# adrianstanea/UnitSpeech

Measured on AMD Instinct MI355X. Metric: mel-frames/sec @ 50 diffusion steps, 80x1024, higher is better.
Workload: dtype f32; 1 GPU; B=1 utterance(s)/GPU, 80x1024 mel, 50 diffusion steps, text+spk CFG (3 score evals/step), full-size decoder (119.1M params, synthetic weights), built-in Philox noise; batch_per_gpu=1, frames=1024, diffusion_steps=50, parallelism=utterance-sharded x1

## Files before the change

unitspeech_amd/csrc/wino4.hip:

```cpp
#include "kernels.h"
#include "pack_f16.h"
#include "wino4_coef.h"

namespace us {

typedef float f32x4 __attribute__((ext_vector_type(4)));
typedef _Float16 half4w __attribute__((ext_vector_type(4)));

namespace {

template <int M> struct Coef;
template <> struct Coef<4> {
  static constexpr int N = 6;
  static constexpr float bt(int i, int j) { return wino4::kBT4[i][j]; }
  static constexpr float at(int i, int j) { return wino4::kAT4[i][j]; }
  static constexpr double g(int i, int j) { return wino4::kG4[i][j]; }
};
template <> struct Coef<2> {
  static constexpr int N = 4;
  static constexpr float bt(int i, int j) { return wino4::kBT2[i][j]; }
  static constexpr float at(int i, int j) { return wino4::kAT2[i][j]; }
  static constexpr double g(int i, int j) { return wino4::kG2[i][j]; }
};

__device__ __forceinline__ void axpy(f32x4& acc, float c, const f32x4& x, bool& first) {
  if (c == 0.f) return;
  if (first) { acc = c == 1.f ? x : (c == -1.f ? -x : x * c); first = false; return; }
  if (c == 1.f) acc += x;
  else if (c == -1.f) acc -= x;
  else acc += x * c;
}

constexpr float kVScale = 0x1p-5f, kVUnscale = 0x1p+5f;

template <int M> struct Bt;
template <> struct Bt<4> {
  __device__ static __forceinline__ void apply(const f32x4 (&d)[6], f32x4 (&o)[6]) {
    using K = Coef<4>;
    static_assert(K::bt(2, 1) == -K::bt(1, 1) && K::bt(2, 3) == -K::bt(1, 3) && K::bt(2, 2) == K::bt(1, 2) && K::bt(1, 4) == 1.f, "symmetric points");
    static_assert(K::bt(4, 1) == -K::bt(3, 1) && K::bt(4, 3) == -K::bt(3, 3) && K::bt(4, 2) == K::bt(3, 2) && K::bt(3, 4) == 1.f, "symmetric points");
    static_assert(K::bt(0, 4) == 1.f && K::bt(5, 5) == 1.f && K::bt(0, 1) == 0.f && K::bt(0, 3) == 0.f && K::bt(5, 2) == 0.f && K::bt(5, 4) == 0.f, "layout");
    o[0] = d[0] * K::bt(0, 0) + (d[2] * K::bt(0, 2) + d[4]);
    o[5] = d[1] * K::bt(5, 1) + (d[3] * K::bt(5, 3) + d[5]);
    const f32x4 e1 = d[2] * K::bt(1, 2) + d[4], o1 = d[1] * K::bt(1, 1) + d[3] * K::bt(1, 3);
    o[1] = e1 + o1;
    o[2] = e1 - o1;
    const f32x4 e2 = d[2] * K::bt(3, 2) + d[4], o2 = d[1] * K::bt(3, 1) + d[3] * K::bt(3, 3);
    o[3] = e2 + o2;
    o[4] = e2 - o2;
  }
};
template <> struct Bt<2> {
  __device__ static __forceinline__ void apply(const f32x4 (&d)[4], f32x4 (&o)[4]) {
    using K = Coef<2>;
    static_assert(K::bt(0, 0) == -1.f && K::bt(0, 2) == 1.f && K::bt(1, 1) == 1.f && K::bt(1, 2) == 1.f && K::bt(2, 1) == -1.f && K::bt(2, 2) == 1.f &&
                      K::bt(3, 1) == -1.f && K::bt(3, 3) == 1.f, "F(2, 3) on {0, +-1, inf}");
    o[0] = d[2] - d[0];
    o[1] = d[2] + d[1];
    o[2] = d[2] - d[1];
    o[3] = d[3] - d[1];
  }
};

template <int MH, int MW, bool GN>
__global__ __launch_bounds__(256) void wino4_input_kernel(const float* __restrict__ x, int x_ld, float* __restrict__ V, int B, int H, int W,
                                                          int C, WinoGnArgs g, unsigned* range_flag) {
  constexpr int NH = Coef<MH>::N, NW = Coef<MW>::N;
  const int C4 = C >> 2;
  const int th = (H + MH - 1) / MH, tw = (W + MW - 1) / MW;
  const int b = blockIdx.y;
  const unsigned per_item = (unsigned)th * tw * C4;
  const long long plane_h = 2LL * B * th * tw * C;
  const unsigned item_bytes = (unsigned)H * W * x_ld * 4u;
  __amdgpu_buffer_rsrc_t rx = __builtin_amdgcn_make_buffer_rsrc((void*)(x + (long long)b * H * W * x_ld), 0, (int)item_bytes, 0x00020000);
  const float* mb = GN ? g.mask + (long long)(b % g.mask_bmod) * g.mask_ld : nullptr;
  const int cg = C / kGroups;
  _Float16* vb = reinterpret_cast<_Float16*>(V) + 2LL * (long long)b * th * tw * C;
  int tc = -1;
  f32x4 sc = {0.f, 0.f, 0.f, 0.f}, sh = sc, te = sc;
  float amax = 0.f;
  for (unsigned i = blockIdx.x * 256u + threadIdx.x; i < per_item; i += gridDim.x * 256u) {
    const unsigned t = i / C4;
    const int c = (int)(i - t * C4) * 4;
    const int ty = (int)(t / tw), tx = (int)(t - (unsigned)ty * tw);
    if (GN && tc != c) {
      tc = c;
      const double cnt = (double)H * W * cg;
      const double mean = stat_read(g.stats, b, c / cg, 0) / cnt;
      double var = stat_read(g.stats, b, c / cg, 1) / cnt - mean * mean;
      if (var < 0) var = 0;
      const float meanf = (float)mean, rstd = (float)(1.0 / sqrt(var + 1e-5));
      const f32x4 ga = *reinterpret_cast<const f32x4*>(g.gamma + c), be = *reinterpret_cast<const f32x4*>(g.beta + c);
      sc = ga * rstd;
      sh = be - sc * meanf;
      te = g.temb ? *reinterpret_cast<const f32x4*>(g.temb + (long long)b * C + c) : f32x4{0.f, 0.f, 0.f, 0.f};
      te *= kVScale;
    }
    unsigned coff[NW];
    float cm[NW];
#pragma unroll
    for (int q = 0; q < NW; ++q) {
      const int ix = MW * tx - 1 + q;
      const bool ok = (unsigned)ix < (unsigned)W;
      coff[q] = ok ? ((unsigned)ix * (unsigned)x_ld + (unsigned)c) * 4u : 0x80000000u;
      if (GN) cm[q] = ok ? mb[ix * g.mask_step] : 0.f;
    }
    f32x4 tr[NH][NW];
#pragma unroll
    for (int r = 0; r < NH; ++r) {
      const int iy = MH * ty - 1 + r;
      const bool rok = (unsigned)iy < (unsigned)H;
      const unsigned roff = rok ? (unsigned)iy * (unsigned)W * (unsigned)x_ld * 4u : 0x80000000u;
      f32x4 d[NW];
#pragma unroll
      for (int q = 0; q < NW; ++q) {
        f32x4 v = __builtin_bit_cast(f32x4, __builtin_amdgcn_raw_buffer_load_b128(rx, (int)((roff + (coff[q] & 0x7fffffffu)) | (coff[q] & 0x80000000u)), 0, 0));
        if (GN) {
          const float m = rok ? cm[q] : 0.f;
#pragma unroll
          for (int k = 0; k < 4; ++k) {
            const float z = v[k] * sc[k] + sh[k];
            const float w = __expf(z);
            const float u = w * (w + 2.f);
            const float mi = z > 20.f ? z : z * (u * __builtin_amdgcn_rcpf(u + 2.f));
            v[k] = (mi * (m * kVScale) + te[k]) * m;
          }
        } else {
          v *= kVScale;
        }
        d[q] = v;
      }
      Bt<MW>::apply(d, tr[r]);
    }
    const unsigned vo = ((unsigned)(ty * tw + tx) * (unsigned)C + (unsigned)c);
    const unsigned ho = 2u * (vo & ~7u) + (vo & 7u);
#pragma unroll
    for (int j = 0; j < NW; ++j) {
      f32x4 col[NH], vv[NH];
#pragma unroll
      for (int r = 0; r < NH; ++r) col[r] = tr[r][j];
      Bt<MH>::apply(col, vv);
#pragma unroll
      for (int ii = 0; ii < NH; ++ii) {
        half4w hi, lo;
#pragma unroll
        for (int k = 0; k < 4; ++k) {
          const float xv = vv[ii][k];
          amax = fmaxf(amax, fabsf(xv));
          const us_half h = (us_half)xv;
          hi[k] = h;
          lo[k] = (us_half)((xv - (float)h) * 2048.f);
        }
        _Float16* pf = vb + (long long)(ii * NW + j) * plane_h;
        *reinterpret_cast<half4w*>(pf + ho) = hi;
        *reinterpret_cast<half4w*>(pf + ho + 8) = lo;
      }
    }
  }
  range_report(range_flag, amax >= kF16Over, kRangeAct);
}

template <int MH, int MW>
__global__ __launch_bounds__(256) void wino4_output_kernel(const float* __restrict__ M, const float* __restrict__ bias, float* __restrict__ out,
                                                           int out_ld, double* __restrict__ stats, int B, int H, int W, int C) {
  using CH = Coef<MH>;
  using CW = Coef<MW>;
  constexpr int NH = CH::N, NW = CW::N;
  __shared__ double s_g[kGroups][2];
  const int C4 = C >> 2;
  const int th = (H + MH - 1) / MH, tw = (W + MW - 1) / MW;
  const int b = blockIdx.y;
  const long long per_item = (long long)th * tw * C4;
  const long long plane = (long long)B * th * tw * C;
  const int cg = C / kGroups;
  if (threadIdx.x < kGroups * 2) s_g[threadIdx.x >> 1][threadIdx.x & 1] = 0.0;
  __syncthreads();
  double t1[4] = {0, 0, 0, 0}, t2[4] = {0, 0, 0, 0};
  int tc = -1;
  auto flush = [&]() {
    if (tc >= 0) {
#pragma unroll
      for (int k = 0; k < 4; ++k) {
        atomicAdd(&s_g[(tc + k) / cg][0], t1[k]);
        atomicAdd(&s_g[(tc + k) / cg][1], t2[k]);
        t1[k] = t2[k] = 0;
      }
    }
  };
  for (unsigned i = blockIdx.x * 256u + threadIdx.x; i < (unsigned)per_item; i += gridDim.x * 256u) {
    const unsigned t = i / (unsigned)C4;
    const int c = (int)(i - t * (unsigned)C4) * 4;
    const int ty = (int)(t / (unsigned)tw);
    const int tx = (int)(t - (unsigned)ty * (unsigned)tw);
    const float* mb = M + (((long long)b * th + ty) * tw + tx) * C + c;
    f32x4 y[MH][MW];
#pragma unroll
    for (int r = 0; r < MH; ++r)
#pragma unroll
      for (int q = 0; q < MW; ++q) y[r][q] = f32x4{0.f, 0.f, 0.f, 0.f};
#pragma unroll
    for (int fi = 0; fi < NH; ++fi) {
      f32x4 m[NW];
#pragma unroll
      for (int fj = 0; fj < NW; ++fj) m[fj] = *reinterpret_cast<const f32x4*>(mb + (long long)(fi * NW + fj) * plane);
#pragma unroll
      for (int q = 0; q < MW; ++q) {
        f32x4 u = {0.f, 0.f, 0.f, 0.f};
        bool first = true;
#pragma unroll
        for (int fj = 0; fj < NW; ++fj) axpy(u, CW::at(q, fj), m[fj], first);
#pragma unroll
        for (int r = 0; r < MH; ++r) {
          bool never = false;
          axpy(y[r][q], CH::at(r, fi), u, never);
        }
      }
    }
    f32x4 bv = {0.f, 0.f, 0.f, 0.f};
    if (bias) bv = *reinterpret_cast<const f32x4*>(bias + c);
    if (stats && tc != c) { flush(); tc = c; }
    float* ob = out + (long long)b * H * W * out_ld + c;
#pragma unroll
    for (int r = 0; r < MH; ++r)
#pragma unroll
      for (int q = 0; q < MW; ++q) {
        const int oy = MH * ty + r, ox = MW * tx + q;
        if (oy < H && ox < W) {
          const f32x4 v = y[r][q] * kVUnscale + bv;
          *reinterpret_cast<f32x4*>(ob + ((long long)oy * W + ox) * out_ld) = v;
          if (stats) {
#pragma unroll
            for (int k = 0; k < 4; ++k) { t1[k] += (double)v[k]; t2[k] += (double)(v[k] * v[k]); }
          }
        }
      }
  }
  if (stats) {
    const int seg = C4 / kGroups;
    const bool wave_merge = (((long long)gridDim.x * 256) % C4) == 0 && seg >= 1 && seg <= 64 && (seg & (seg - 1)) == 0 && (64 % seg) == 0 &&
                            (C4 % 64 == 0 || 64 % C4 == 0);
    if (wave_merge) {
      double s1 = (t1[0] + t1[1]) + (t1[2] + t1[3]), s2 = (t2[0] + t2[1]) + (t2[2] + t2[3]);
      for (int off = 1; off < seg; off <<= 1) {
        s1 += __shfl_xor(s1, off);
        s2 += __shfl_xor(s2, off);
      }
      const int lane = threadIdx.x & 63;
      if ((lane & (seg - 1)) == 0 && tc >= 0) {
        atomicAdd(&s_g[tc / cg][0], s1);
        atomicAdd(&s_g[tc / cg][1], s2);
      }
    } else {
      flush();
    }
    __syncthreads();
    if (threadIdx.x < kGroups * 2)
      stat_add(stats, b, threadIdx.x >> 1, threadIdx.x & 1, blockIdx.x, s_g[threadIdx.x >> 1][threadIdx.x & 1]);
  }
}

template <int MH, int MW>
__global__ __launch_bounds__(256) void wino4_pack_kernel(const float* __restrict__ src, _Float16* __restrict__ dst, int Cout, int Cin,
                                                         unsigned* range_flag) {
  using CH = Coef<MH>;
  using CW = Coef<MW>;
  constexpr int NH = CH::N, NW = CW::N;
  bool over = false;
  const long long total = (long long)(Cin / 8) * Cout;
  const long long fstride = (long long)Cin * Cout * 2;
  for (long long i = blockIdx.x * 256LL + threadIdx.x; i < total; i += (long long)gridDim.x * 256) {
    const int g4 = (int)(i & 3);
    const long long rn = i >> 2;
    const int n = (int)(rn % Cout), kc = (int)(rn / Cout);
    const int k0 = kc * 32 + g4 * 8;
    float gk[8][9];
#pragma unroll
    for (int kk = 0; kk < 8; ++kk) {
      const float* gs = src + ((long long)n * Cin + k0 + kk) * 9;
#pragma unroll
      for (int t = 0; t < 9; ++t) gk[kk][t] = gs[t];
    }
    _Float16* d = dst + (rn * 32 + g4 * 8) * 2;
#pragma unroll
    for (int fi = 0; fi < NH; ++fi)
#pragma unroll
      for (int fj = 0; fj < NW; ++fj) {
        pk_half8 hi, lo;
#pragma unroll
        for (int kk = 0; kk < 8; ++kk) {
          double u = 0.0;
#pragma unroll
          for (int a = 0; a < 3; ++a)
#pragma unroll
            for (int bb = 0; bb < 3; ++bb) {
              const double cf = CH::g(fi, a) * CW::g(fj, bb);
              if (cf != 0.0) u += cf * (double)gk[kk][a * 3 + bb];
            }
          us_half h, l;
          split_f16x3((float)u, h, l, over);
          hi[kk] = h;
          lo[kk] = l;
        }
        *reinterpret_cast<pk_half8*>(d + (long long)(fi * NW + fj) * fstride) = hi;
        *reinterpret_cast<pk_half8*>(d + (long long)(fi * NW + fj) * fstride + 8) = lo;
      }
  }
  range_report(range_flag, over, kRangeWeight);
}

int grid_for(long long per_item) {
  long long blocks = (per_item + 255) / 256;
  return (int)(blocks < 1 ? 1 : (blocks > 4096 ? 4096 : blocks));
}

}

bool wino4_form_ok(int form) { return form == 44 || form == 24; }
int wino4_freqs(int form) { return form == 44 ? 36 : (form == 24 ? 24 : 0); }
void wino4_tiles(int form, int H, int W, int* th, int* tw) {
  const int mh = form / 10, mw = form % 10;
  *th = (H + mh - 1) / mh;
  *tw = (W + mw - 1) / mw;
}

hipError_t launch_wino4_input(int form, const float* x, int x_ld, float* V, int B, int H, int W, int C, const WinoGnArgs* gn, hipStream_t s) {
  if (!wino4_form_ok(form) || C % 8 != 0 || x_ld % 4 != 0 || B > 65535) return hipErrorInvalidValue;
  if ((long long)H * W * x_ld * 4 >= (1LL << 31) || (long long)H * W * C >= (1LL << 30)) return hipErrorInvalidValue;
  WinoGnArgs g{};
  if (gn) {
    g = *gn;
    if (!g.stats || !g.gamma || !g.beta || !g.mask || g.h_out || x_ld != C || C % kGroups != 0 || (C / kGroups) % 4 != 0) return hipErrorInvalidValue;
    if (g.mask_bmod < 1) g.mask_bmod = 1;
  }
  int th, tw;
  wino4_tiles(form, H, W, &th, &tw);
  const dim3 grid(grid_for((long long)th * tw * (C / 4)), B);
  unsigned* rf = current_range_flag();
  if (form == 44) {
    if (gn) hipLaunchKernelGGL((wino4_input_kernel<4, 4, true>), grid, dim3(256), 0, s, x, x_ld, V, B, H, W, C, g, rf);
    else hipLaunchKernelGGL((wino4_input_kernel<4, 4, false>), grid, dim3(256), 0, s, x, x_ld, V, B, H, W, C, g, rf);
  } else {
    if (gn) hipLaunchKernelGGL((wino4_input_kernel<2, 4, true>), grid, dim3(256), 0, s, x, x_ld, V, B, H, W, C, g, rf);
    else hipLaunchKernelGGL((wino4_input_kernel<2, 4, false>), grid, dim3(256), 0, s, x, x_ld, V, B, H, W, C, g, rf);
  }
  return hipGetLastError();
}

hipError_t launch_wino4_output(int form, const float* M, const float* bias, float* out, int out_ld, double* stats, int B, int H, int W, int C,
                               hipStream_t s) {
  if (!wino4_form_ok(form) || C % 4 != 0 || out_ld % 4 != 0 || C % kGroups != 0 || B > 65535) return hipErrorInvalidValue;
  int th, tw;
  wino4_tiles(form, H, W, &th, &tw);
  if ((long long)th * tw * (C / 4) >= (1LL << 31)) return hipErrorInvalidValue;
  const dim3 grid(grid_for((long long)th * tw * (C / 4)), B);
  if (form == 44) hipLaunchKernelGGL((wino4_output_kernel<4, 4>), grid, dim3(256), 0, s, M, bias, out, out_ld, stats, B, H, W, C);
  else hipLaunchKernelGGL((wino4_output_kernel<2, 4>), grid, dim3(256), 0, s, M, bias, out, out_ld, stats, B, H, W, C);
  return hipGetLastError();
}

hipError_t launch_wino4_pack_weight(int form, const float* src, float* dst, int Cout, int Cin, hipStream_t s) {
  if (!wino4_form_ok(form) || Cin % 32 != 0) return hipErrorInvalidValue;
  const long long total = (long long)Cout * Cin / 8;
  long long blocks = (total + 255) / 256;
  if (blocks > 8192) blocks = 8192;
  unsigned* rf = current_range_flag();
  if (form == 44) hipLaunchKernelGGL((wino4_pack_kernel<4, 4>), dim3((int)blocks), dim3(256), 0, s, src, reinterpret_cast<_Float16*>(dst), Cout, Cin, rf);
  else hipLaunchKernelGGL((wino4_pack_kernel<2, 4>), dim3((int)blocks), dim3(256), 0, s, src, reinterpret_cast<_Float16*>(dst), Cout, Cin, rf);
  return hipGetLastError();
}

}
```

Baseline: 3205 mel-frames/s.

## Stage Winograd input patches in LDS and pair hi/lo stores via permlane swap

The Winograd input transform now gives each workgroup a spatial patch of tiles plus a 32-channel slab. It loads the overlapping halo region once into shared memory, applying GroupNorm+Mish there, instead of each thread reloading overlapping 6x6 windows from global memory and recomputing the activation per overlap. Lanes in the two wave halves swap hi/lo f16 halves with permlane32_swap so each lane writes one 16-byte store instead of two 8-byte stores. This adds LDS use, a barrier, a fixed grid shape and FP-contract control in the Bt transform, which may affect occupancy and numerics.

```diff
diff --git a/unitspeech_amd/csrc/wino4.hip b/unitspeech_amd/csrc/wino4.hip
--- a/unitspeech_amd/csrc/wino4.hip
+++ b/unitspeech_amd/csrc/wino4.hip
@@ -2,10 +2,14 @@
 #include "pack_f16.h"
 #include "wino4_coef.h"
 
+#include <type_traits>
+
 namespace us {
 
 typedef float f32x4 __attribute__((ext_vector_type(4)));
 typedef _Float16 half4w __attribute__((ext_vector_type(4)));
+typedef unsigned u32x2 __attribute__((ext_vector_type(2)));
+typedef unsigned u32x4 __attribute__((ext_vector_type(4)));
 
 namespace {
 
@@ -35,13 +39,24 @@
 
 template <int M> struct Bt;
 template <> struct Bt<4> {
+  template <bool kScaledInput = false>
   __device__ static __forceinline__ void apply(const f32x4 (&d)[6], f32x4 (&o)[6]) {
     using K = Coef<4>;
     static_assert(K::bt(2, 1) == -K::bt(1, 1) && K::bt(2, 3) == -K::bt(1, 3) && K::bt(2, 2) == K::bt(1, 2) && K::bt(1, 4) == 1.f, "symmetric points");
     static_assert(K::bt(4, 1) == -K::bt(3, 1) && K::bt(4, 3) == -K::bt(3, 3) && K::bt(4, 2) == K::bt(3, 2) && K::bt(3, 4) == 1.f, "symmetric points");
     static_assert(K::bt(0, 4) == 1.f && K::bt(5, 5) == 1.f && K::bt(0, 1) == 0.f && K::bt(0, 3) == 0.f && K::bt(5, 2) == 0.f && K::bt(5, 4) == 0.f, "layout");
     o[0] = d[0] * K::bt(0, 0) + (d[2] * K::bt(0, 2) + d[4]);
-    o[5] = d[1] * K::bt(5, 1) + (d[3] * K::bt(5, 3) + d[5]);
+    if constexpr (kScaledInput) {
+      f32x4 t;
+      {
+#pragma clang fp contract(off)
+        const f32x4 p = d[3] * K::bt(5, 3);
+        t = p + d[5];
+      }
+      o[5] = d[1] * K::bt(5, 1) + t;
+    } else {
+      o[5] = d[1] * K::bt(5, 1) + (d[3] * K::bt(5, 3) + d[5]);
+    }
     const f32x4 e1 = d[2] * K::bt(1, 2) + d[4], o1 = d[1] * K::bt(1, 1) + d[3] * K::bt(1, 3);
     o[1] = e1 + o1;
     o[2] = e1 - o1;
@@ -62,29 +77,59 @@
   }
 };
 
+template <int MH, int MW> struct Patch {
+  static constexpr int PH = MH == 4 ? 2 : 5, PW = 8;
+  static constexpr int RH = PH * MH + 2, RW = PW * MW + 2;
+  static constexpr int kPix = RH * RW;
+  static constexpr int kSlab = 32;
+  static constexpr int kPixStride = 9;
+  static constexpr int kThreads = PH * 64;
+  static constexpr int kIter = (kPix * 8 + kThreads - 1) / kThreads;
+  static_assert(kPix * kPixStride * 16 <= 64 * 1024, "two workgroups share a CU's LDS");
+};
+
 template <int MH, int MW, bool GN>
-__global__ __launch_bounds__(256) void wino4_input_kernel(const float* __restrict__ x, int x_ld, float* __restrict__ V, int B, int H, int W,
-                                                          int C, WinoGnArgs g, unsigned* range_flag) {
+__global__ __launch_bounds__((Patch<MH, MW>::kThreads)) void wino4_input_kernel(const float* __restrict__ x, int x_ld, float* __restrict__ V, int B,
+                                                                               int H, int W, int C, WinoGnArgs g, unsigned* range_flag, int slabs,
+                                                                               int patches_w) {
+  using P = Patch<MH, MW>;
   constexpr int NH = Coef<MH>::N, NW = Coef<MW>::N;
-  const int C4 = C >> 2;
+  __shared__ f32x4 s_d[P::kPix * P::kPixStride];
   const int th = (H + MH - 1) / MH, tw = (W + MW - 1) / MW;
   const int b = blockIdx.y;
-  const unsigned per_item = (unsigned)th * tw * C4;
+  const int slab = (int)(blockIdx.x % (unsigned)slabs);
+  const int patch = (int)(blockIdx.x / (unsigned)slabs);
+  const int pty = patch / patches_w, ptx = patch - pty * patches_w;
+  const int tid = threadIdx.x;
   const long long plane_h = 2LL * B * th * tw * C;
   const unsigned item_bytes = (unsigned)H * W * x_ld * 4u;
   __amdgpu_buffer_rsrc_t rx = __builtin_amdgcn_make_buffer_rsrc((void*)(x + (long long)b * H * W * x_ld), 0, (int)item_bytes, 0x00020000);
-  const float* mb = GN ? g.mask + (long long)(b % g.mask_bmod) * g.mask_ld : nullptr;
-  const int cg = C / kGroups;
   _Float16* vb = reinterpret_cast<_Float16*>(V) + 2LL * (long long)b * th * tw * C;
-  int tc = -1;
-  f32x4 sc = {0.f, 0.f, 0.f, 0.f}, sh = sc, te = sc;
-  float amax = 0.f;
-  for (unsigned i = blockIdx.x * 256u + threadIdx.x; i < per_item; i += gridDim.x * 256u) {
-    const unsigned t = i / C4;
-    const int c = (int)(i - t * C4) * 4;
-    const int ty = (int)(t / tw), tx = (int)(t - (unsigned)ty * tw);
-    if (GN && tc != c) {
-      tc = c;
+  {
+    const int q = tid & 7;
+    const int c = slab * P::kSlab + q * 4;
+    const bool cok = c < C;
+    const int slot = (q >> 1) + 4 * (q & 1);
+    const float* mb = GN ? g.mask + (long long)(b % g.mask_bmod) * g.mask_ld : nullptr;
+    const int y0 = pty * (P::PH * MH) - 1, x0 = ptx * (P::PW * MW) - 1;
+    f32x4 v[P::kIter];
+    float pm[P::kIter];
+#pragma unroll
+    for (int k = 0; k < P::kIter; ++k) {
+      const int p = (tid + k * P::kThreads) >> 3;
+      const int py = p / P::RW, px = p - py * P::RW;
+      const int iy = y0 + py, ix = x0 + px;
+      const bool ok = cok && (unsigned)iy < (unsigned)H && (unsigned)ix < (unsigned)W && p < P::kPix;
+      const unsigned off = ok ? (((unsigned)iy * (unsigned)W + (unsigned)ix) * (unsigned)x_ld + (unsigned)c) * 4u : 0x80000000u;
+      v[k] = __builtin_bit_cast(f32x4, __builtin_amdgcn_raw_buffer_load_b128(rx, (int)off, 0, 0));
+      if (GN) {
+        const float mv = mb[min(max(ix, 0), W - 1) * g.mask_step];
+        pm[k] = ok ? mv : 0.f;
+      }
+    }
+    f32x4 sc = {0.f, 0.f, 0.f, 0.f}, sh = sc, te = sc;
+    if (GN && cok) {
+      const int cg = C / kGroups;
       const double cnt = (double)H * W * cg;
       const double mean = stat_read(g.stats, b, c / cg, 0) / cnt;
       double var = stat_read(g.stats, b, c / cg, 1) / cnt - mean * mean;
@@ -96,44 +141,44 @@
       te = g.temb ? *reinterpret_cast<const f32x4*>(g.temb + (long long)b * C + c) : f32x4{0.f, 0.f, 0.f, 0.f};
       te *= kVScale;
     }
-    unsigned coff[NW];
-    float cm[NW];
-#pragma unroll
-    for (int q = 0; q < NW; ++q) {
-      const int ix = MW * tx - 1 + q;
-      const bool ok = (unsigned)ix < (unsigned)W;
-      coff[q] = ok ? ((unsigned)ix * (unsigned)x_ld + (unsigned)c) * 4u : 0x80000000u;
-      if (GN) cm[q] = ok ? mb[ix * g.mask_step] : 0.f;
-    }
+#pragma unroll
+    for (int k = 0; k < P::kIter; ++k) {
+      const int p = (tid + k * P::kThreads) >> 3;
+      f32x4 d = v[k];
+      if (GN) {
+        const float m = pm[k];
+#pragma unroll
+        for (int kk = 0; kk < 4; ++kk) {
+          const float z = d[kk] * sc[kk] + sh[kk];
+          const float w = __expf(z);
+          const float u = w * (w + 2.f);
+          const float mi = z > 20.f ? z : z * (u * __builtin_amdgcn_rcpf(u + 2.f));
+          d[kk] = (mi * (m * kVScale) + te[kk]) * m;
+        }
+      } else {
+        d *= kVScale;
+      }
+      if (p < P::kPix) s_d[p * P::kPixStride + slot] = d;
+    }
+  }
+  __syncthreads();
+  const int lane = tid & 63, trow = tid >> 6;
+  const int tcol = (lane & 31) >> 2, oct = lane & 3, odd = lane >> 5;
+  const int ty = pty * P::PH + trow, tx = ptx * P::PW + tcol;
+  const int c8 = slab * P::kSlab + oct * 8;
+  float amax = 0.f;
+  if (ty < th && tx < tw && c8 < C) {
+    const f32x4* sp = s_d + ((trow * MH) * P::RW + tcol * MW) * P::kPixStride + oct + 4 * odd;
     f32x4 tr[NH][NW];
 #pragma unroll
     for (int r = 0; r < NH; ++r) {
-      const int iy = MH * ty - 1 + r;
-      const bool rok = (unsigned)iy < (unsigned)H;
-      const unsigned roff = rok ? (unsigned)iy * (unsigned)W * (unsigned)x_ld * 4u : 0x80000000u;
       f32x4 d[NW];
 #pragma unroll
-      for (int q = 0; q < NW; ++q) {
-        f32x4 v = __builtin_bit_cast(f32x4, __builtin_amdgcn_raw_buffer_load_b128(rx, (int)((roff + (coff[q] & 0x7fffffffu)) | (coff[q] & 0x80000000u)), 0, 0));
-        if (GN) {
-          const float m = rok ? cm[q] : 0.f;
-#pragma unroll
-          for (int k = 0; k < 4; ++k) {
-            const float z = v[k] * sc[k] + sh[k];
-            const float w = __expf(z);
-            const float u = w * (w + 2.f);
-            const float mi = z > 20.f ? z : z * (u * __builtin_amdgcn_rcpf(u + 2.f));
-            v[k] = (mi * (m * kVScale) + te[k]) * m;
-          }
-        } else {
-          v *= kVScale;
-        }
-        d[q] = v;
-      }
-      Bt<MW>::apply(d, tr[r]);
-    }
-    const unsigned vo = ((unsigned)(ty * tw + tx) * (unsigned)C + (unsigned)c);
-    const unsigned ho = 2u * (vo & ~7u) + (vo & 7u);
+      for (int q = 0; q < NW; ++q) d[q] = sp[(r * P::RW + q) * P::kPixStride];
+      Bt<MW>::template apply<true>(d, tr[r]);
+    }
+    const unsigned vo = (unsigned)(ty * tw + tx) * (unsigned)C + (unsigned)c8;
+    const unsigned ho = 2u * vo + 8u * (unsigned)odd;
 #pragma unroll
     for (int j = 0; j < NW; ++j) {
       f32x4 col[NH], vv[NH];
@@ -151,9 +196,12 @@
           hi[k] = h;
           lo[k] = (us_half)((xv - (float)h) * 2048.f);
         }
+        const u32x2 hu = __builtin_bit_cast(u32x2, hi), lu = __builtin_bit_cast(u32x2, lo);
+        const u32x2 s0 = __builtin_amdgcn_permlane32_swap(hu[0], lu[0], false, false);
+        const u32x2 s1 = __builtin_amdgcn_permlane32_swap(hu[1], lu[1], false, false);
+        const u32x4 o = {s0[0], s1[0], s0[1], s1[1]};
         _Float16* pf = vb + (long long)(ii * NW + j) * plane_h;
-        *reinterpret_cast<half4w*>(pf + ho) = hi;
-        *reinterpret_cast<half4w*>(pf + ho + 8) = lo;
+        *reinterpret_cast<u32x4*>(pf + ho) = o;
       }
     }
   }
@@ -334,16 +382,19 @@
   }
   int th, tw;
   wino4_tiles(form, H, W, &th, &tw);
-  const dim3 grid(grid_for((long long)th * tw * (C / 4)), B);
   unsigned* rf = current_range_flag();
-  if (form == 44) {
-    if (gn) hipLaunchKernelGGL((wino4_input_kernel<4, 4, true>), grid, dim3(256), 0, s, x, x_ld, V, B, H, W, C, g, rf);
-    else hipLaunchKernelGGL((wino4_input_kernel<4, 4, false>), grid, dim3(256), 0, s, x, x_ld, V, B, H, W, C, g, rf);
-  } else {
-    if (gn) hipLaunchKernelGGL((wino4_input_kernel<2, 4, true>), grid, dim3(256), 0, s, x, x_ld, V, B, H, W, C, g, rf);
-    else hipLaunchKernelGGL((wino4_input_kernel<2, 4, false>), grid, dim3(256), 0, s, x, x_ld, V, B, H, W, C, g, rf);
-  }
-  return hipGetLastError();
+  auto run = [&](auto mh, auto mw) {
+    using P = Patch<decltype(mh)::value, decltype(mw)::value>;
+    const int slabs = (C + P::kSlab - 1) / P::kSlab, pw = (tw + P::PW - 1) / P::PW, ph = (th + P::PH - 1) / P::PH;
+    const long long blocks = (long long)ph * pw * slabs;
+    if (blocks >= (1LL << 31)) return hipErrorInvalidValue;
+    const dim3 grid((unsigned)blocks, B), block(P::kThreads);
+    if (gn) hipLaunchKernelGGL((wino4_input_kernel<decltype(mh)::value, decltype(mw)::value, true>), grid, block, 0, s, x, x_ld, V, B, H, W, C, g, rf, slabs, pw);
+    else hipLaunchKernelGGL((wino4_input_kernel<decltype(mh)::value, decltype(mw)::value, false>), grid, block, 0, s, x, x_ld, V, B, H, W, C, g, rf, slabs, pw);
+    return hipGetLastError();
+  };
+  if (form == 44) return run(std::integral_constant<int, 4>{}, std::integral_constant<int, 4>{});
+  return run(std::integral_constant<int, 2>{}, std::integral_constant<int, 4>{});
 }
 
 hipError_t launch_wino4_output(int form, const float* M, const float* bias, float* out, int out_ld, double* stats, int B, int H, int W, int C,
```

Result: no change. 3225 mel-frames/s, median of 6 (+0.6%).
